# iyioon/NYPC-Yacht-Auction

Hardware: AMD Instinct MI355X
Metric: MCTS node-expansions/sec/GPU @4096 envs x100 sims; episodes/sec 1-8 GPU (higher is better)
Workload: dtype f32

## Files before the change

nypc-yacht-auction_amd/csrc/yk_engine.hip:

```cpp
#include <math.h>

#include <algorithm>
#include <vector>

#include "yk_api.h"
#include "yk_common.h"
#include "yk_engine_dev.h"
#include "yk_forced.h"
#include "yk_net.h"

#define YK_MAX_GROUPS 8

using namespace yk;

namespace {


struct PwPlan {
    int nleaf, nop, root;
    uint16_t start[64], len[64];
    uint8_t a[64], b[64];
};
constexpr int pw_build(PwPlan& p, int start, int n) {
    if (n <= 128) {
        p.start[p.nleaf] = (uint16_t)start;
        p.len[p.nleaf] = (uint16_t)n;
        return p.nleaf++;
    }
    int n2 = n / 2;
    n2 -= n2 % 8;
    const int l = pw_build(p, start, n2);
    const int r = pw_build(p, start + n2, n - n2);
    p.a[p.nop] = (uint8_t)l;
    p.b[p.nop] = (uint8_t)r;
    return 64 + p.nop++;
}
constexpr PwPlan make_plan() {
    PwPlan p{};
    p.root = pw_build(p, 0, ASIZE);
    return p;
}
static __constant__ PwPlan c_pw = make_plan();
static_assert(make_plan().nleaf <= 64 && make_plan().nop <= 64, "pairwise plan too large");
constexpr bool plan_is_butterfly() {
    const PwPlan p = make_plan();
    if (p.nleaf != 32 || p.nop != 31) return false;
    int first[128] = {}, cnt[128] = {};
    for (int i = 0; i < p.nleaf; i++) {
        if (p.start[i] % 8 != 0 || p.len[i] < 8 || p.len[i] > 128) return false;
        if (i > 0 && p.start[i] != p.start[i - 1] + p.len[i - 1]) return false;
        first[i] = i;
        cnt[i] = 1;
    }
    for (int o = 0; o < p.nop; o++) {
        const int a = p.a[o], b = p.b[o];
        if (cnt[a] != cnt[b] || first[a] + cnt[a] != first[b] || first[a] % (2 * cnt[a]) != 0) return false;
        first[64 + o] = first[a];
        cnt[64 + o] = 2 * cnt[a];
    }
    return p.root == 64 + p.nop - 1 && cnt[p.root] == 32;
}
static_assert(plan_is_butterfly(), "numpy's pairwise tree for 3226 is no longer a perfect 32-leaf tree");
constexpr int pw_gmax() {
    const PwPlan p = make_plan();
    int g = 0;
    for (int i = 0; i < p.nleaf; i++) g = p.len[i] / 8 > g ? p.len[i] / 8 : g;
    return g;
}
constexpr int pw_tmax() {
    const PwPlan p = make_plan();
    int t = 0;
    for (int i = 0; i < p.nleaf; i++) t = p.len[i] % 8 > t ? p.len[i] % 8 : t;
    return t;
}
constexpr int PW_GMAX = pw_gmax();
constexpr int PW_TMAX = pw_tmax() > 0 ? pw_tmax() : 1;
constexpr int pw_lmax() {
    const PwPlan p = make_plan();
    int l = 0;
    for (int i = 0; i < p.nleaf; i++) l = p.len[i] > l ? p.len[i] : l;
    return l;
}
static_assert(NCOMB > pw_lmax(), "two category starts could share a leaf of the pairwise plan");
static_assert(PF_WCAP % 8 == 0 && PF_WCAP >= 16 && GAMES_PER_BLOCK * PF_WCAP * 4 <= 40 * 1024,
              "the prior window: whole float4 pairs, a slot per category, 16 waves per CU");

struct ValidQ {
    int mode;
    int n;
    uint32_t used;
    __device__ __forceinline__ bool operator()(int a) const {
        if (mode == 1) return a < NBID;
        if (mode != 0 || a < NBID) return false;
        const int base = a - NBID, cat = base / NCOMB, ci = base - cat * NCOMB;
        if ((used >> cat) & 1u) return false;
        if (n >= 10) return true;
        if (n == 5) return ci == 0;
        return c_tab.comb_max[ci] < n;
    }
};
__device__ __forceinline__ ValidQ valid_q(const YkS& s) {
    ValidQ q;
    const int round = s_round(s), phase = s_phase(s);
    const uint64_t wa = s_pw(s, 0, 0);
    q.n = __builtin_amdgcn_readfirstlane(wa_n(wa));
    q.used = __builtin_amdgcn_readfirstlane((uint32_t)wa_used(wa));
    q.mode = __builtin_amdgcn_readfirstlane((phase == 0 && round != 13) ? 1 : (phase == 1 && q.n >= 5) ? 0 : -1);
    return q;
}


__device__ __forceinline__ void wave_sync() {
    __builtin_amdgcn_fence(__ATOMIC_ACQ_REL, "workgroup");
    __builtin_amdgcn_wave_barrier();
}

__device__ __forceinline__ float wave_max(float v) {
    v = fmaxf(v, xlane<32>(v));
    v = fmaxf(v, xlane<16>(v));
    v = fmaxf(v, xlane<8>(v));
    v = fmaxf(v, xlane<4>(v));
    v = fmaxf(v, xlane<2>(v));
    return fmaxf(v, xlane<1>(v));
}
__device__ __forceinline__ float softmax_p(float x, float m, float lse) { return exp_acc(x - m - lse); }
__device__ __forceinline__ float wave_sumf(float v) {
    v += xlane<32>(v);
    v += xlane<16>(v);
    v += xlane<8>(v);
    v += xlane<4>(v);
    v += xlane<2>(v);
    return v + xlane<1>(v);
}
__device__ __forceinline__ int wave_min_i(int v) {
    v = min(v, xlane<32>(v));
    v = min(v, xlane<16>(v));
    v = min(v, xlane<8>(v));
    v = min(v, xlane<4>(v));
    v = min(v, xlane<2>(v));
    return min(v, xlane<1>(v));
}

struct PyV {
    double v;
    uint32_t t;
};
__device__ __forceinline__ PyV pv_update(PyV q, uint32_t n, PyV v) {
    PyV prod, sum, out;
    if (q.t == T_F32) prod = PyV{(double)((float)n * (float)q.v), T_F32};
    else prod = PyV{(double)n * q.v, q.t};
    if (prod.t == T_F32 || v.t == T_F32) sum = PyV{(double)((float)prod.v + (float)v.v), T_F32};
    else if (prod.t == T_F64 || v.t == T_F64) sum = PyV{prod.v + v.v, T_F64};
    else sum = PyV{prod.v + v.v, T_INT};
    if (sum.t == T_F32) out = PyV{(double)((float)sum.v / (float)(n + 1)), T_F32};
    else out = PyV{sum.v / (double)(n + 1), T_F64};
    return out;
}

__global__ void k_lut(float* sq, float* sqe) {
    const int i = blockIdx.x * blockDim.x + threadIdx.x;
    if (i >= LUT_N) return;
    sq[i] = (float)sqrt((double)i);
    sqe[i] = (float)sqrt((double)i + 1e-8);
}

__global__ void k_reset(EngDev d, int start_games, uint32_t env_base) {
    const int e = blockIdx.x * blockDim.x + threadIdx.x;
    if (e >= d.E) return;
    for (int t = e; t < d.T; t += d.E) {
        d.node_count[t] = d.node_count[d.T + t] = 0;
        d.edge_count[t] = d.edge_count[d.T + t] = 0;
        d.arena_top[t] = 0;
        d.gen[t] = 0;
        d.cur_round[t] = 0;
        d.root_c[2 * t] = make_uint4(0, 0, 0, 0);
        d.root_c[2 * t + 1] = make_uint4(0, 0, RV_OFF, 0);
    }
#pragma unroll
    for (int k = 0; k < GST; k++) d.gstats[(long)e * GST + k] = 0;
    if (!start_games) return;
    d.env_id[e] = env_base + (uint32_t)e;
    Stream rs{d.seed, d.env_id[e], 0};
    YkS s;
#pragma unroll
    for (int k = 0; k < 8; k++) s.w[k] = 0;
    s.w[0] = 1ull | NO_BIDS;
    new_round_rolls(s, rs);
    st_state(d.board + e, s);
    d.cur[e] = 1;
    d.ctr[e] = rs.ctr;
    d.done[e] = 0;
    d.nmoves[e] = 0;
    d.rec_voff[(long)e * (d.M + 1)] = 0;
}

__global__ __launch_bounds__(256) void k_move_begin(EngDev d, int move, int external_root) {
    const int lane = threadIdx.x & 63;
    const int e = d.e_lo + blockIdx.x * GAMES_PER_BLOCK + (threadIdx.x >> 6);
    if (e >= d.e_hi) return;
    const int t = tree_of(d, e);
    if (lane == 0) {
        d.root_c[2 * t] = make_uint4(0, 0, 0, 0);
        d.root_c[2 * t + 1] = make_uint4(0, 0, RV_OFF, 0);
    }
    if (!external_root) {
        if (d.done[e]) return;
        const YkS b = ld_state(d.board + e);
        const YkS r = canonical(b, d.cur[e]);
        const bool idle = d.arena && (d.cur[e] == d.seat[e] ? d.arena_agent : d.arena_opp) != YK_PLAYER_MCTS;
        if (lane == 0) {
            st_state(d.root + e, r);
            d.rec_ctr[((long)e * d.M + move) * 2] = d.ctr[e];
            d.idle[e] = idle ? 1 : 0;
        }
        if (idle) return;
    } else if (lane == 0) {
        d.idle[e] = 0;
    }
    const YkS r = ld_state(d.root + e);
    const int rr = s_round(r);
    const int cr = d.cur_round[t];
    if (rr == cr) return;
    if (rr < cr) {
        if (lane == 0) atomicOr(d.err, ERR_ROUND);
        return;
    }
    const int g = d.gen[t], h = g ^ 1;
    uint32_t* hx = d.hidx[h] + (long)t * d.HCAP;
    for (int i = lane; i < d.HCAP; i += 64) hx[i] = 0;
    const NodeRec* src = d.nodes[g] + (long)t * d.NCAP;
    NodeRec* dst = d.nodes[h] + (long)t * d.NCAP;
    const Edge* esrc = d.edges[g] + (long)t * d.ECAP;
    Edge* edst = d.edges[h] + (long)t * d.ECAP;
    float* P = d.arenaP + (long)t * d.AE;
    uint16_t* S = d.arenaS + (long)t * d.AE;
    const uint32_t cnt = d.node_count[g * d.T + t];
    uint32_t nn = 0, ne = 0, top = 0;
    wave_sync();
// ... 444 lines not shown
            }
            wave_sync();
            int soff = -8;
            float4 sv = make_float4(0.f, 0.f, 0.f, 0.f);
            if (fast == 2) {
                const int c = st <= NBID ? 0 : (st - NBID + NCOMB - 1) / NCOMB;
                const int o = NBID + NCOMB * c - st;
                if (c < NCAT && o < nl) {
                    const float pc = win[c];
                    soff = o;
                    sv = make_float4((o & 3) == 0 ? pc : 0.f, (o & 3) == 1 ? pc : 0.f, (o & 3) == 2 ? pc : 0.f,
                                     (o & 3) == 3 ? pc : 0.f);
                }
            }
#pragma unroll
            for (int j = 0; j < PW_GMAX; j++) {
                const int o = 8 * j + 4 * h;
                float4 w = make_float4(0.f, 0.f, 0.f, 0.f);
                if (fast == 1) {
                    const int i = st + o - wbase;
                    if (j < G && (unsigned)i < (unsigned)wlen) w = *reinterpret_cast<const float4*>(win + i);
                } else if (j < G && o == (soff & ~3)) {
                    w = sv;
                }
                q[j] = w;
            }
#pragma unroll
            for (int r = 0; r < PW_TMAX; r++) {
                const int o = 8 * G + r, i = st + o - wbase;
                float w = 0.f;
                if (h == 0 && r < R) {
                    if (fast == 1) {
                        if ((unsigned)i < (unsigned)wlen) w = win[i];
                    } else if (o == soff) {
                        w = win[wslot(st + o)];
                    }
                }
                qt[r] = w;
            }
            masked = true;
        } else if (d.prior == 0) {
            const float* x = d.logits + (long)e * PI_LD + st;
            static_assert(NBID % 4 == 2 && NCOMB % 4 == 0, "category starts are 2 mod 4");
            const bool score10 = valid.mode == 0 && valid.n >= 10;
#pragma unroll
            for (int j = 0; j < PW_GMAX; j++) {
                const int a = st + 8 * j + 4 * h;
                bool v0, v1, v2, v3;
                if (score10) {
                    const int b0 = a - NBID, b2 = a + 2 - NBID;
                    const bool lo = j < G && b0 >= 0 && !((valid.used >> ((unsigned)b0 / NCOMB)) & 1u);
                    const bool hi = j < G && b2 >= 0 && !((valid.used >> ((unsigned)b2 / NCOMB)) & 1u);
                    v0 = v1 = lo;
                    v2 = v3 = hi;
                } else {
                    v0 = j < G && valid(a);
                    v1 = j < G && valid(a + 1);
                    v2 = j < G && valid(a + 2);
                    v3 = j < G && valid(a + 3);
                }
                float4 x4 = make_float4(0.f, 0.f, 0.f, 0.f);
                if (v0 || v1 || v2 || v3) x4 = *reinterpret_cast<const float4*>(x + 8 * j + 4 * h);
                q[j] = make_float4(v0 ? softmax_p(x4.x, mx, lse) : 0.f, v1 ? softmax_p(x4.y, mx, lse) : 0.f,
                                   v2 ? softmax_p(x4.z, mx, lse) : 0.f, v3 ? softmax_p(x4.w, mx, lse) : 0.f);
            }
#pragma unroll
            for (int r = 0; r < PW_TMAX; r++)
                qt[r] = (h == 0 && r < R && valid(st + 8 * G + r)) ? softmax_p(x[8 * G + r], mx, lse) : 0.f;
            masked = true;
        } else {
#pragma unroll
            for (int j = 0; j < PW_GMAX; j++) {
                const int a = st + 8 * j + 4 * h;
                q[j] = j < G ? make_float4(hash_prior_pi(hsh, a), hash_prior_pi(hsh, a + 1), hash_prior_pi(hsh, a + 2),
                                           hash_prior_pi(hsh, a + 3))
                             : make_float4(0.f, 0.f, 0.f, 0.f);
            }
#pragma unroll
            for (int r = 0; r < PW_TMAX; r++) qt[r] = (h == 0 && r < R) ? hash_prior_pi(hsh, st + 8 * G + r) : 0.f;
        }
#pragma unroll
        for (int j = 0; j < PW_GMAX; j++) {
            const int a = st + 8 * j + 4 * h;
            if (j < G && !masked) {
                if (!valid(a)) q[j].x = 0.f;
                if (!valid(a + 1)) q[j].y = 0.f;
                if (!valid(a + 2)) q[j].z = 0.f;
                if (!valid(a + 3)) q[j].w = 0.f;
            }
        }
#pragma unroll
        for (int r = 0; r < PW_TMAX; r++)
            if (h == 0 && r < R && !masked && !valid(st + 8 * G + r)) qt[r] = 0.f;
        if (rec) {
            float* rpi = d.rec_pi + rslot * ASIZE;
#pragma unroll
            for (int j = 0; j < PW_GMAX; j++)
                if (j < G) *reinterpret_cast<float4*>(rpi + st + 8 * j + 4 * h) = q[j];
#pragma unroll
            for (int r = 0; r < PW_TMAX; r++)
                if (h == 0 && r < R) rpi[st + 8 * G + r] = qt[r];
            if (lane == 0) {
                d.rec_v[rslot] = v;
                st_state(d.rec_leaf + rslot, s);
            }
        }
        float4 racc = q[0];
#pragma unroll
        for (int j = 1; j < PW_GMAX; j++)
            if (j < G) {
                racc.x += q[j].x;
                racc.y += q[j].y;
                racc.z += q[j].z;
                racc.w += q[j].w;
            }
        const float half = (racc.x + racc.y) + (racc.z + racc.w);
        const float other = xlane<1>(half);
        float lsum = h == 0 ? half + other : other + half;
#pragma unroll
        for (int r = 0; r < PW_TMAX; r++)
            if (r < R) lsum += qt[r];
        lsum = __builtin_bit_cast(float, dpp_mov<0xA0>(__builtin_bit_cast(uint32_t, lsum)));
        float y = xlane<2>(lsum);
        lsum = (lane & 2) ? y + lsum : lsum + y;
        y = xlane<4>(lsum);
        lsum = (lane & 4) ? y + lsum : lsum + y;
        y = xlane<8>(lsum);
        lsum = (lane & 8) ? y + lsum : lsum + y;
        y = xlane<16>(lsum);
        lsum = (lane & 16) ? y + lsum : lsum + y;
        y = xlane<32>(lsum);
        lsum = (lane & 32) ? y + lsum : lsum + y;
        const float sum = lsum;
        const int VP = pad4(V);
        const uint32_t off = d.arena_top[t];
        const uint32_t nid = d.node_count[g * d.T + t];
        bool ok = true;
        if ((int64_t)off + VP > d.AE) {
            if (lane == 0) atomicOr(d.err, ERR_ARENA);
            ok = false;
        }
        if (nid >= (uint32_t)d.NCAP) {
            if (lane == 0) atomicOr(d.err, ERR_NODES);
            ok = false;
        }
        if (ok) {
            float* P = d.arenaP + (long)t * d.AE + off;
            uint16_t* S = d.arenaS + (long)t * d.AE + off;
            const float inv_fallback = V > 0 ? 1.0f / (float)V : 0.0f;
            const float* __restrict__ xr = d.logits + (long)e * PI_LD;
            const float sqe0 = (float)sqrt((double)0u + 1e-8);
            float fb = -INFINITY;
            int fj = 0x7FFFFFFF;
            for (int j0 = lane; j0 < VP; j0 += 256) {
                float xa[4];
                int aa[4];
#pragma unroll
                for (int u = 0; u < 4; u++) {
                    const int j = j0 + 64 * u;
                    aa[u] = j < V ? compact_to_action(vi, j) : 0;
                    xa[u] = (d.prior == 0 && !fast && j < V) ? xr[aa[u]] : 0.f;
                }
#pragma unroll
                for (int u = 0; u < 4; u++) {
                    const int j = j0 + 64 * u;
                    if (j < VP) {
                        float p = 0.0f;
                        if (j < V) {
                            const float pa = fast            ? win[wslot(aa[u])]
                                             : d.prior == 0 ? softmax_p(xa[u], mx, lse)
                                                            : hash_prior_pi(hsh, aa[u]);
                            p = sum > 0.0f ? pa / sum : inv_fallback;
                            const float u0 = (d.c32 * p) * sqe0;
                            if (u0 > fb) {
                                fb = u0;
                                fj = j;
                            }
                        }
                        P[j] = p;
                        S[j] = 0;
                    }
                }
            }
            wave_argmax_step(fb, fj);
            if (lane == 0) {
                NodeRec r;
#pragma unroll
                for (int i = 0; i < 8; i++) r.key[i] = s.w[i];
                r.hash = ihsh;
                r.vinfo = pack_vinfo(vi);
                r.p_off = off;
                r.nvalid = (uint32_t)V;
                r.Ns = 0;
                r.first_j = (uint32_t)fj;
                d.nodes[g][(long)t * d.NCAP + nid] = r;
                if (!insert_index(d, g, t, ihsh, nid)) atomicOr(d.err, ERR_HASH);
            }
            end_id = nid + 1;
            if (lane == 0) {
                d.node_count[g * d.T + t] = nid + 1;
                d.arena_top[t] = off + (uint32_t)VP;
                unsigned long long* gs = reinterpret_cast<unsigned long long*>(d.gstats + (long)e * GST);
                atomicAdd(gs + 0, 1ull);
                atomicAdd(gs + 3, (unsigned long long)V);
                atomicAdd(gs + (fast == 1 ? 9 : fast == 2 ? 10 : 11), 1ull);
                atomicMax(gs + 4, (unsigned long long)(nid + 1));
                atomicMax(gs + 6, (unsigned long long)(off + (uint32_t)VP));
            }
        }
        res = PyV{-(double)v, T_F32};
    } else {
        end_id = d.end_node[e];
    }
    const int depth = d.path_len[e];
    if (depth > 0) {
        NodeRec* nodes = d.nodes[g] + (long)t * d.NCAP;
        Edge* edges = d.edges[g] + (long)t * d.ECAP;
        uint16_t* Sb = d.arenaS + (long)t * d.AE;
        const uint64_t* path = d.path + (long)e * MAXD;
        const uint32_t ne0 = d.edge_count[g * d.T + t];
        uint64_t pe = 0;
        uint16_t sl = 0;
        if (lane < depth) {
            pe = path[lane];
            sl = Sb[pe >> 32];
        }
        const uint32_t pnext = __shfl((uint32_t)pe, (lane + 1) & 63, 64);
        const uint32_t cnode = lane + 1 < depth ? (pnext & ~PATH_DET) + 1 : end_id;
        const uint32_t cbits = ((uint32_t)pe & PATH_DET) ? cnode << 2 : 0u;
        const bool is_new = lane < depth && sl == 0;
        const uint64_t bal = __ballot(is_new);
        const uint32_t eid = ne0 + (uint32_t)__popcll(bal & ((1ull << lane) - 1));
        const uint32_t ne1 = ne0 + (uint32_t)__popcll(bal);
        if (lane < depth) {
            PyV v = res;
            if ((depth - 1 - lane) & 1) v.v = -v.v;
            if (sl) {
                Edge& ed = edges[sl - 1];
                const PyV q = pv_update(PyV{ed.Q, edge_kind(ed.tag)}, ed.N, v);
                ed.Q = q.v;
                ed.tag = q.t | cbits;
                ed.N += 1;
            } else if (eid < (uint32_t)d.ECAP && eid < 65535u) {
                edges[eid] = Edge{v.v, 1u, v.t | cbits};
                Sb[pe >> 32] = (uint16_t)(eid + 1);
            } else {
                atomicOr(d.err, ERR_EDGES);
            }
            nodes[(uint32_t)pe & ~PATH_DET].Ns += 1;
        }
        if (lane == 0) {
            d.edge_count[g * d.T + t] = ne1;
            atomicMax(reinterpret_cast<unsigned long long*>(d.gstats + (long)e * GST) + 5, (unsigned long long)ne1);
            if (is_new && eid < (uint32_t)d.ECAP && eid < 65535u) {
                const uint32_t n = d.root_c[2 * t + 1].z;
                if (n != RV_OFF) {
                    const uint32_t j = (uint32_t)(pe >> 32) - d.root_c[2 * t].y;
                    if (n < (uint32_t)RV_CAP) {
                        d.rv[(long)t * RV_CAP + n] = j | ((eid + 1) << 12);
                        d.root_c[2 * t + 1].z = n + 1;
                    } else {
                        d.root_c[2 * t + 1].z = RV_OFF;
                    }
                }
            }
        }
    }
}

__global__ __launch_bounds__(256) void k_root_sort(EngDev d) {
    constexpr int PT = (RO_CAP + 255) / 256;
    __shared__ uint64_t sk[RO_K];
    __shared__ uint32_t hist[256];
    __shared__ int s_nid, s_need;
    __shared__ uint32_t s_nv, s_cnt;
    __shared__ uint64_t s_prefix;
    const int e = d.e_lo + (int)blockIdx.x;
    if (e >= d.e_hi || d.done[e] || d.idle[e] || !(d.c32 > 0.f)) return;
    const int tid = threadIdx.x, lane = tid & 63;
    const int t = tree_of(d, e);
    const int g = d.gen[t];
    const uint4 rc0 = d.root_c[2 * t];
    if (tid < 64) {
        int nid = rc0.x ? (int)rc0.x - 1 : -1;
        if (nid < 0) {
            const YkS r = ld_state(d.root + e);
            nid = lookup(d, g, t, r, index_hash(r));
        }
        if (tid == 0) {
            s_nid = nid;
            s_nv = 0;
            s_cnt = 0;
        }
    }
    __syncthreads();
    const int nid = s_nid;
    if (nid < 0) return;
    const NodeRec& nd = d.nodes[g][(long)t * d.NCAP + nid];
    const int V = (int)nd.nvalid;
    const uint32_t p_off = nd.p_off;
    if (V <= 256 || V > RO_CAP) return;
    const float* P = d.arenaP + (long)t * d.AE + p_off;
    const uint16_t* S = d.arenaS + (long)t * d.AE + p_off;
    uint32_t* rv = d.rv + (long)t * RV_CAP;
    uint64_t key[PT];
#pragma unroll
    for (int i = 0; i < PT; i++) {
        const int j = tid + 256 * i;
        key[i] = 0;
        if (j < V) {
            key[i] = ((uint64_t)__float_as_uint(P[j]) << 16) | (uint32_t)(0xFFFFu - (uint32_t)j);
            const uint16_t sl = S[j];
            if (sl) {
                const uint32_t pos = atomicAdd(&s_nv, 1u);
                if (pos < (uint32_t)RV_CAP) rv[pos] = (uint32_t)j | ((uint32_t)sl << 12);
            }
        }
    }
    const int K = V < d.ro_k ? V : d.ro_k;
    uint64_t thr = 1;
    if (V > K) {
        uint64_t prefix = 0, mask = 0;
        int need = K;
        for (int sh = 40; sh >= 0; sh -= 8) {
            hist[tid] = 0;
            __syncthreads();
#pragma unroll
            for (int i = 0; i < PT; i++)
                if (key[i] && (key[i] & mask) == prefix) atomicAdd(&hist[(uint32_t)(key[i] >> sh) & 255u], 1u);
            __syncthreads();
            if (tid < 64) {
                const uint32_t h0 = hist[4 * lane], h1 = hist[4 * lane + 1], h2 = hist[4 * lane + 2], h3 = hist[4 * lane + 3];
                const uint32_t own = h0 + h1 + h2 + h3;
                uint32_t suf = own;
#pragma unroll
// ... 494 lines not shown
                hipLaunchKernelGGL(k_root_sort, dim3((unsigned)(d.e_hi - d.e_lo)), bb, 0, st[g], d);
                YK_LAUNCHED();
                select(d, st[g]);
                YK_LAUNCHED();
            }
            if (timed && eng->prof_stride > 1) prof_mark(eng, g, -1, st[g]);
        }
    }
    for (int g = 0; g < G; g++) prof_mark(eng, g, -1, st[g]);
    return YK_OK;
}
}

extern "C" {


int yk_engine_create(yk_engine_t** out, const yk_engine_config_t* cfg, yk_net_t* net) {
    if (!out || !cfg) return YK_ERR_ARG;
    if (cfg->n_envs <= 0 || cfg->sims < 1 || cfg->max_moves < 1 || cfg->max_moves > 4096) return YK_ERR_ARG;
    if (cfg->prior == 0 && !net) return YK_ERR_ARG;
    if (cfg->prior != 0 && cfg->prior != 1) return YK_ERR_ARG;
    if (!(cfg->dirichlet_alpha >= 0.0) || !(cfg->dirichlet_eps >= 0.0 && cfg->dirichlet_eps <= 1.0)) return YK_ERR_ARG;
    std::unique_ptr<yk_engine> eng(new yk_engine());
    eng->cfg = *cfg;
    eng->net = net;
    EngDev& d = eng->d;
    d.E = cfg->n_envs;
    d.sims = cfg->sims;
    d.c32 = (float)cfg->cpuct;
    d.temp_threshold = cfg->temp_threshold;
    d.prior = cfg->prior;
    d.M = cfg->max_moves;
    d.NCAP = 6 * cfg->sims + 64;
    int hcap = 1;
    while (hcap < 2 * d.NCAP) hcap <<= 1;
    d.HCAP = hcap;
    d.ECAP = std::min(4 * d.NCAP, 65535);
    if (cfg->arena_entries > 0) {
        d.AE = (cfg->arena_entries + 3) & ~3LL;
    } else {
        const int64_t worst = (int64_t)d.NCAP * 3024;
        size_t free_b = 0, total_b = 0;
        (void)hipMemGetInfo(&free_b, &total_b);
        const double need = (double)worst * 6.0 * cfg->n_envs * (cfg->dual_trees ? 2 : 1);
        d.AE = (need < 0.6 * (double)free_b) ? worst : (int64_t)cfg->sims * 9000 + 65536;
    }
    d.VCAP = (int)record_vcap(cfg->max_moves, cfg->sims);
    d.rec_pred = cfg->record_predictions ? 1 : 0;
    d.max_exp = cfg->record_predictions ? std::max(cfg->max_expansions, 1) : 0;
    d.rec_stride = std::max(cfg->record_stride, 1);
    d.e_lo = 0;
    d.e_hi = d.E;
    d.T = cfg->dual_trees ? 2 * d.E : d.E;
    d.dual = 0;
    eng->net2 = net;
    int G = cfg->groups > 0 ? cfg->groups : ((cfg->prior == 0 && cfg->n_envs >= 8192) ? 2 : 1);
    G = std::max(1, std::min({G, YK_MAX_GROUPS, (cfg->n_envs + GROUP_ALIGN - 1) / GROUP_ALIGN}));
    eng->ngroups = G;
constexpr int YK_FPARTS_MAX = 4;
    {
        int cus = 256, dev = 0;
        if (hipGetDevice(&dev) == hipSuccess) (void)hipDeviceGetAttribute(&cus, hipDeviceAttributeMultiprocessorCount, dev);
        const int tiles = G * (((cfg->n_envs + G - 1) / G + 15) / 16);
        d.fparts = 1;
        while (d.fparts * 2 <= YK_FPARTS_MAX && tiles * d.fparts * 2 <= cus) d.fparts *= 2;
        eng->fparts_single = d.fparts;
        if (cfg->dual_trees && G == 1 && cfg->prior == 0 && 2 * tiles <= cus) {
            eng->fparts_dual = 1;
            while (eng->fparts_dual * 2 <= YK_FPARTS_MAX && 2 * tiles * eng->fparts_dual * 2 <= cus) eng->fparts_dual *= 2;
        }
    }
    const size_t R = ((size_t)cfg->n_envs + d.rec_stride - 1) / d.rec_stride;
    const size_t E = (size_t)d.E, T = (size_t)d.T;
#define A(p, n) YK_TRY(eng->mem.alloc(&(p), (n)))
    for (int g = 0; g < 2; g++) {
        A(d.nodes[g], T * d.NCAP);
        A(d.hidx[g], T * d.HCAP);
        A(d.edges[g], T * d.ECAP);
    }
    A(d.node_count, 2 * T);
    A(d.edge_count, 2 * T);
    A(d.arenaP, T * (size_t)d.AE);
    A(d.arenaS, T * (size_t)d.AE);
    A(d.arena_top, T);
    A(d.gen, T);
    A(d.cur_round, T);
    A(d.root_c, 2 * T);
    A(d.rv, T * RV_CAP);
    A(d.ro_j, T * RO_K);
    A(d.ro_p, T * RO_K);
    A(d.board, E);
    A(d.cur, E);
    A(d.ctr, E);
    A(d.env_id, E);
    A(d.done, E);
    A(d.nmoves, E);
    A(d.root, E);
    A(d.leaf_state, E);
    A(d.leaf_hash, E);
    A(d.leaf_flag, E);
    A(d.path, E * MAXD);
    A(d.path_len, E);
    A(d.end_node, E);
    A(d.res_v, E);
    A(d.res_t, E);
    A(eng->vpred, E);
    A(eng->mlse, E * (size_t)d.fparts);
    A(eng->lut_sq, (size_t)LUT_N);
    A(eng->lut_sqe, (size_t)LUT_N);
    A(d.rec_state, E * d.M);
    A(d.rec_info, E * d.M * 8);
    A(d.rec_ctr, E * d.M * 2);
    A(d.rec_val, E * d.M);
    A(d.rec_visits, E * (size_t)d.VCAP);
    A(d.rec_voff, E * (d.M + 1));
    A(d.final_r, E);
    A(d.final_cur, E);
    A(d.final_tot, 2 * E);
    A(d.seat, E);
    A(d.idle, E);
    A(d.gstats, E * GST);
    A(d.err, 1);
    A(eng->done_count, 1);
    A(eng->mcts_env, E);
    if (d.prior == 0) {
        A(eng->logits, E * (size_t)PI_LD);
    }
    eng->root_values = cfg->record_root_values != 0;
    eng->noise = cfg->dirichlet_alpha > 0.0 && cfg->dirichlet_eps > 0.0;
    eng->nz.alpha = cfg->dirichlet_alpha;
    eng->nz.eps = cfg->dirichlet_eps;
    if (eng->noise) {
        A(eng->nz.noised, E);
        if (d.rec_pred) {
            A(eng->nz.prior_before, R * (size_t)d.M * ASIZE);
            A(eng->nz.prior_after, R * (size_t)d.M * ASIZE);
        }
    }
    if (d.rec_pred) {
        A(d.rec_pi, R * (size_t)d.max_exp * ASIZE);
        A(d.rec_v, R * (size_t)d.max_exp);
        A(d.rec_leaf, R * (size_t)d.max_exp);
    }
#undef A
    if (hipHostMalloc((void**)&eng->host_done, sizeof(int32_t)) != hipSuccess) return YK_ERR_NOMEM;
    {
        const char* ev = getenv("YK_ROOT_SCAN");
        eng->root_scan = !(ev && ev[0] == '0');
        const char* ek = getenv("YK_ROOT_K");
        d.ro_k = ek ? std::max(1, std::min(RO_K, atoi(ek))) : RO_K;
        const char* en = getenv("YK_NODE_SUMMARY");
        d.node_summary = (en && en[0] == '0') ? 0 : 1;
        const char* ep = getenv("YK_PRIOR_FAST");
        d.prior_fast = (ep && ep[0] == '0') ? 0 : 1;
        const char* es = getenv("YK_SPLIT_DESCENT");
        eng->split_descent = es && es[0] == '1';
    }
    if (G > 1) {
        if (hipEventCreateWithFlags(&eng->ev_fork, hipEventDisableTiming) != hipSuccess) return YK_ERR_HIP;
        for (int g = 0; g < G; g++)
            if (hipStreamCreateWithFlags(&eng->gs[g], hipStreamNonBlocking) != hipSuccess ||
                hipEventCreateWithFlags(&eng->ev_join[g], hipEventDisableTiming) != hipSuccess ||
                hipEventCreateWithFlags(&eng->ev_fwd[g], hipEventDisableTiming) != hipSuccess)
                return YK_ERR_HIP;
    }
    if (eng->fparts_dual > 0) {
        if (hipStreamCreateWithFlags(&eng->dstream, hipStreamNonBlocking) != hipSuccess ||
            hipEventCreateWithFlags(&eng->ev_d0, hipEventDisableTiming) != hipSuccess ||
            hipEventCreateWithFlags(&eng->ev_d1, hipEventDisableTiming) != hipSuccess)
            return YK_ERR_HIP;
    }
    d.logits = eng->logits;
    d.vpred = eng->vpred;
    d.mlse = eng->mlse;
    d.lut_sq = eng->lut_sq;
    d.lut_sqe = eng->lut_sqe;
    hipLaunchKernelGGL(k_lut, dim3(LUT_N / 256), dim3(256), 0, 0, eng->lut_sq, eng->lut_sqe);
    YK_LAUNCHED();
    YK_HIP(hipMemset(d.err, 0, sizeof(uint32_t)));
    YK_HIP(hipMemset(d.done, 0, E));
    YK_HIP(hipMemset(d.idle, 0, E));
    YK_HIP(hipMemset(d.leaf_state, 0, sizeof(yk_state_t) * E));
    std::vector<uint32_t> ids(E);
    for (size_t i = 0; i < E; i++) ids[i] = (uint32_t)i;
    YK_HIP(hipMemcpy(eng->mcts_env, ids.data(), sizeof(uint32_t) * E, hipMemcpyHostToDevice));
    YK_HIP(hipDeviceSynchronize());
    *out = eng.release();
    return YK_OK;
}

int yk_engine_destroy(yk_engine_t* eng) {
    delete eng;
    return YK_OK;
}

}

namespace {
bool playout_full(uint64_t seed, uint32_t env_base, int move, double full_prob) {
    return u53(philox_u64(philox4x32_10(seed, (uint32_t)move, env_base, 0u, PHILOX_PLAYOUT))) < full_prob;
}

int play_batch(yk_engine* eng, uint64_t seed, uint32_t env_base, hipStream_t s) {
    EngDev& d = eng->d;
    d.seed = seed;
    const int G = eng->ngroups;
    hipStream_t st[YK_MAX_GROUPS];
    EngDev dg[YK_MAX_GROUPS];
    for (int g = 0; g < G; g++) {
        st[g] = G == 1 ? s : eng->gs[g];
        dg[g] = G == 1 ? d : group_dev(eng, g);
    }
    const dim3 bb(256);
    YK_HIP(hipMemsetAsync(d.err, 0, sizeof(uint32_t), s));
    YK_HIP(hipMemsetAsync(d.hidx[0], 0, sizeof(uint32_t) * (size_t)d.T * d.HCAP, s));
    const bool noise = eng->noise && !d.arena;
    const bool root_values = eng->root_values && !d.arena;
    const bool capped = eng->fast_sims > 0 && !d.arena;
    eng->have_priors = false;
    eng->fast_moves = 0;
    const bool forcing = eng->forced_k > 0.0 && !d.arena;
    const ForcedDev fd{eng->forced_k, eng->cfg.cpuct};
    if (root_values)
        YK_HIP(hipMemsetAsync(d.rec_info, 0, sizeof(int32_t) * (size_t)d.E * d.M * 8, s));
    if (noise && eng->nz.prior_after) {
        const size_t nb = sizeof(float) * (((size_t)d.E + d.rec_stride - 1) / d.rec_stride) * (size_t)d.M * ASIZE;
        YK_HIP(hipMemsetAsync(eng->nz.prior_before, 0, nb, s));
        YK_HIP(hipMemsetAsync(eng->nz.prior_after, 0, nb, s));
    }
    hipLaunchKernelGGL(k_reset, dim3((d.E + 255) / 256), dim3(256), 0, s, d, 1, env_base);
    YK_LAUNCHED();
    if (G > 1) {
        YK_HIP(hipEventRecord(eng->ev_fork, s));
        for (int g = 0; g < G; g++) YK_HIP(hipStreamWaitEvent(st[g], eng->ev_fork, 0));
    }
    eng->have_records = false;
    for (int move = 0; move < d.M; move++) {
        for (int g = 0; g < G; g++) {
            prof_mark(eng, g, KC_MOVE_BEGIN, st[g]);
            hipLaunchKernelGGL(k_move_begin, game_grid(dg[g]), bb, 0, st[g], dg[g], move, 0);
            YK_LAUNCHED();
        }
        const bool fast = capped && !playout_full(seed, env_base, move, eng->full_prob);
        eng->fast_moves += fast;
        if (!d.arena || d.arena_agent == YK_PLAYER_MCTS || d.arena_opp == YK_PLAYER_MCTS) {
            int rc = run_sims(eng, G, st, fast ? eng->fast_sims : d.sims, d.env_id, d.ctr, noise && !fast ? move : -1,
                              forcing && !fast ? &fd : nullptr);
            if (rc) return rc;
        }
        for (int g = 0; g < G; g++) {
            prof_mark(eng, g, KC_MOVE_END, st[g]);
            if (forcing && !fast && eng->forced_prune)
                hipLaunchKernelGGL((k_move_end<true, ForcedDev>), game_grid(dg[g]), bb, 0, st[g], dg[g], move, 0, fd);
            else
                hipLaunchKernelGGL((k_move_end<false>), game_grid(dg[g]), bb, 0, st[g], dg[g], move,
                                   fast ? YK_REC_FAST : 0);
            YK_LAUNCHED();
            if (root_values) {
                prof_mark(eng, g, KC_ROOT_VALUE, st[g]);
                const RootValDev rv{move};
                const int rc = yk_launch_root_value(&dg[g], sizeof(dg[g]), &rv, sizeof(rv), st[g]);
                if (rc) return rc;
            }
            prof_mark(eng, g, -1, st[g]);
            if (G > 1) {
                YK_HIP(hipEventRecord(eng->ev_join[g], st[g]));
                YK_HIP(hipStreamWaitEvent(s, eng->ev_join[g], 0));
            }
        }
        hipLaunchKernelGGL(k_count_done, dim3(1), dim3(1024), 0, s, d.done, d.E, eng->done_count);
        YK_LAUNCHED();
        YK_HIP(hipMemcpyAsync(eng->host_done, eng->done_count, sizeof(int32_t), hipMemcpyDeviceToHost, s));
        YK_HIP(hipStreamSynchronize(s));
        prof_collect(eng);
        if (*eng->host_done >= d.E) break;
    }
    hipLaunchKernelGGL(k_finalize, dim3((unsigned)(((long)d.E * d.M + 255) / 256)), dim3(256), 0, s, d);
    YK_LAUNCHED();
    eng->have_records = true;
    eng->have_priors = noise && eng->nz.prior_after;
    return check_errors(eng, s);
}
}

extern "C" {

int yk_selfplay(yk_engine_t* eng, uint64_t seed, uint32_t env_base, void* stream) {
    if (!eng) return YK_ERR_ARG;
    eng->d.arena = 0;
    eng->have_arena = false;
    return play_batch(eng, seed, env_base, as_stream(stream));
}

int yk_engine_set_playout_cap(yk_engine_t* eng, int fast_sims, double full_prob) {
    if (!eng || fast_sims < 0) return YK_ERR_ARG;
    if (fast_sims > 0 && (fast_sims < 2 || fast_sims > eng->d.sims || !(full_prob >= 0.0 && full_prob <= 1.0)))
        return YK_ERR_ARG;
    eng->fast_sims = fast_sims;
    eng->full_prob = full_prob;
    return YK_OK;
}

int yk_engine_set_forced_playouts(yk_engine_t* eng, double k, int prune) {
    if (!eng || !(k >= 0.0) || std::isinf(k) || (prune != 0 && prune != 1)) return YK_ERR_ARG;
    eng->forced_k = k;
    eng->forced_prune = prune != 0;
    return YK_OK;
// ... 291 lines not shown
```

Baseline: 31.68 million.

## Stage softmax priors through LDS window in two halves for slow-path expansions

When the prior window cannot hold the whole action vector, the pairwise-sum leaves are now written into the LDS window in two passes, split at the tree's midpoint. Each pass reads priors from LDS instead of recomputing softmax from global logits. When every category is open (n>=10) the pass maps compact indices to actions arithmetically and emits float4 stores. Otherwise it finds the split point by binary search. This mode becomes the default, at the cost of extra wave syncs and more complex index logic.

```diff
diff --git a/nypc-yacht-auction_amd/csrc/yk_engine.hip b/nypc-yacht-auction_amd/csrc/yk_engine.hip
--- a/nypc-yacht-auction_amd/csrc/yk_engine.hip
+++ b/nypc-yacht-auction_amd/csrc/yk_engine.hip
@@ -74,6 +74,13 @@
     return t;
 }
 constexpr int PW_GMAX = pw_gmax();
+constexpr int pw_gmin() {
+    const PwPlan p = make_plan();
+    int g = PW_GMAX;
+    for (int i = 0; i < p.nleaf; i++) g = p.len[i] / 8 < g ? p.len[i] / 8 : g;
+    return g;
+}
+constexpr int PW_GMIN = pw_gmin();
 constexpr int PW_TMAX = pw_tmax() > 0 ? pw_tmax() : 1;
 constexpr int pw_lmax() {
     const PwPlan p = make_plan();
@@ -84,6 +91,21 @@
 static_assert(NCOMB > pw_lmax(), "two category starts could share a leaf of the pairwise plan");
 static_assert(PF_WCAP % 8 == 0 && PF_WCAP >= 16 && GAMES_PER_BLOCK * PF_WCAP * 4 <= 40 * 1024,
               "the prior window: whole float4 pairs, a slot per category, 16 waves per CU");
+constexpr int PW_NLEAF = make_plan().nleaf;
+constexpr int PW_SPLIT = make_plan().start[PW_NLEAF / 2];
+static_assert(PW_SPLIT % 8 == 0 && PW_SPLIT <= PF_WCAP && ASIZE - PW_SPLIT <= PF_WCAP,
+              "both halves of the pairwise tree fit the prior window, float4s aligned");
+static_assert(PW_SPLIT > NBID && (PW_SPLIT - NBID) / NCOMB < NCAT, "the split lies inside a category's block");
+constexpr int PW_SPLIT_CAT = (PW_SPLIT - NBID) / NCOMB, PW_SPLIT_COMB = (PW_SPLIT - NBID) % NCOMB;
+constexpr int pw_leaf2() {
+    const PwPlan p = make_plan();
+    int i = 0;
+    while (ASIZE - p.start[i] > PF_WCAP) i++;
+    return i;
+}
+constexpr int PW_LEAF2 = pw_leaf2(), PW_BASE2 = make_plan().start[PW_LEAF2];
+static_assert(PW_LEAF2 <= PW_NLEAF / 2 && PW_BASE2 % 8 == 0 && PW_BASE2 <= PW_SPLIT - (PW_SPLIT_COMB & 3),
+              "the second piece holds the right half and the group the split cuts");
 
 struct ValidQ {
     int mode;
@@ -834,24 +856,79 @@
             const float sqe0 = (float)sqrt((double)0u + 1e-8);
             float fb = -INFINITY;
             int fj = 0x7FFFFFFF;
-            for (int j0 = lane; j0 < VP; j0 += 256) {
+            const bool staged = d.prior_fast >= 2 && !fast && V > 0;
+            const bool quad = staged && valid.mode == 0 && valid.n >= 10;
+            int jA = 0;
+            if (staged) {
+                if (quad) {
+                    const uint32_t un = ~valid.used & ((1u << NCAT) - 1u);
+                    jA = NCOMB * __builtin_popcount(un & ((1u << PW_SPLIT_CAT) - 1u)) +
+                         (((un >> PW_SPLIT_CAT) & 1u) ? (PW_SPLIT_COMB & ~3) : 0);
+                } else {
+                    int lo = 0, hi = V;
+                    while (lo < hi) {
+                        const int mid = (lo + hi) >> 1;
+                        if (compact_to_action(vi, mid) < PW_SPLIT) lo = mid + 1;
+                        else hi = mid;
+                    }
+                    jA = __builtin_amdgcn_readfirstlane(lo);
+                }
+            }
+            const int nhalf = staged ? 2 : 1;
+            for (int hf = 0; hf < nhalf; hf++) {
+            const int jlo = hf ? jA : 0, jhi = (staged && !hf) ? jA : VP;
+            if (staged) {
+                wbase = hf ? PW_BASE2 : 0;
+                if (hf) wave_sync();
+                if (hf ? leaf >= PW_LEAF2 : leaf < PW_NLEAF / 2) {
+                    float* wl = win + (st - wbase);
+#pragma unroll
+                    for (int j = 0; j < PW_GMAX; j++)
+                        if (j < PW_GMIN || j < G) *reinterpret_cast<float4*>(wl + 8 * j + 4 * h) = q[j];
+#pragma unroll
+                    for (int r = 0; r < PW_TMAX; r++)
+                        if (h == 0 && r < R) wl[8 * G + r] = qt[r];
+                }
+                wave_sync();
+            }
+            for (int j = jlo + 4 * lane; quad && j < jhi; j += 256) {
+                const int ci = j / NCOMB;
+                const float* w = win + (NBID + NCOMB * (int)((vi.cats >> (4 * ci)) & 0xF) + (j - ci * NCOMB) - wbase);
+                const float2 w01 = *reinterpret_cast<const float2*>(w), w23 = *reinterpret_cast<const float2*>(w + 2);
+                const float pa4[4] = {w01.x, w01.y, w23.x, w23.y};
+                float p4[4];
+#pragma unroll
+                for (int u = 0; u < 4; u++) {
+                    const float pa = pa4[u];
+                    const float p = sum > 0.0f ? pa / sum : inv_fallback;
+                    const float u0 = (d.c32 * p) * sqe0;
+                    if (u0 > fb) {
+                        fb = u0;
+                        fj = j + u;
+                    }
+                    p4[u] = p;
+                }
+                *reinterpret_cast<float4*>(P + j) = make_float4(p4[0], p4[1], p4[2], p4[3]);
+                *reinterpret_cast<uint2*>(S + j) = make_uint2(0u, 0u);
+            }
+            for (int j0 = jlo + lane; !quad && j0 < jhi; j0 += 256) {
                 float xa[4];
                 int aa[4];
 #pragma unroll
                 for (int u = 0; u < 4; u++) {
                     const int j = j0 + 64 * u;
                     aa[u] = j < V ? compact_to_action(vi, j) : 0;
-                    xa[u] = (d.prior == 0 && !fast && j < V) ? xr[aa[u]] : 0.f;
+                    xa[u] = (d.prior == 0 && !fast && !staged && j < V) ? xr[aa[u]] : 0.f;
                 }
 #pragma unroll
                 for (int u = 0; u < 4; u++) {
                     const int j = j0 + 64 * u;
-                    if (j < VP) {
+                    if (j < jhi) {
                         float p = 0.0f;
                         if (j < V) {
-                            const float pa = fast            ? win[wslot(aa[u])]
-                                             : d.prior == 0 ? softmax_p(xa[u], mx, lse)
-                                                            : hash_prior_pi(hsh, aa[u]);
+                            const float pa = (fast || staged) ? win[wslot(aa[u])]
+                                             : d.prior == 0   ? softmax_p(xa[u], mx, lse)
+                                                              : hash_prior_pi(hsh, aa[u]);
                             p = sum > 0.0f ? pa / sum : inv_fallback;
                             const float u0 = (d.c32 * p) * sqe0;
                             if (u0 > fb) {
@@ -863,6 +940,7 @@
                         S[j] = 0;
                     }
                 }
+            }
             }
             wave_argmax_step(fb, fj);
             if (lane == 0) {
@@ -1663,7 +1741,7 @@
         const char* en = getenv("YK_NODE_SUMMARY");
         d.node_summary = (en && en[0] == '0') ? 0 : 1;
         const char* ep = getenv("YK_PRIOR_FAST");
-        d.prior_fast = (ep && ep[0] == '0') ? 0 : 1;
+        d.prior_fast = !ep ? 2 : (ep[0] == '0' && !ep[1]) ? 0 : (ep[0] == '1' && !ep[1]) ? 1 : 2;
         const char* es = getenv("YK_SPLIT_DESCENT");
         eng->split_descent = es && es[0] == '1';
     }
```

Result: faster. 32.52 million, median of 6 (+2.7%).
